# apache/incubator-predictionio

Measured on NVIDIA H100. Metric: ALS iterations/sec, higher is better.
Workload: dtype f32

## Files before the change

incubator-predictionio_b200/csrc/als_lockstep.cuh:

```cuda
#pragma once
#include <cuda_runtime.h>
#include <stdint.h>

namespace pio {

template <int N>
struct LsLayout {
  static constexpr int NBK = N / 16;
  static constexpr int NOFF = NBK * (NBK - 1) / 2;
  static constexpr int DIAG0 = NOFF * 256;
  static constexpr int SIZE = DIAG0 + NBK * 136;
  static constexpr int STRIDE = SIZE + ((SIZE % 32) == 16 ? 0 : (48 - SIZE % 32) % 32);
  __host__ __device__ static constexpr int swz(int rr) { return ((rr >> 1) & 1) * 2 + ((rr >> 2) & 1); }
  __host__ __device__ static constexpr int offd_base(int rb, int cb) { return (rb * (rb - 1) / 2 + cb) * 256; }
  __host__ __device__ static constexpr int offd(int rb, int cb, int rr, int cc) {
    return offd_base(rb, cb) + rr * 16 + 4 * ((cc >> 2) ^ swz(rr)) + (cc & 3);
  }
  __host__ __device__ static constexpr int diag(int rb, int rr, int cc) { return DIAG0 + rb * 136 + rr * (rr + 1) / 2 + cc; }
  __host__ __device__ static constexpr int at(int r, int c) {
    return (r >> 4) == (c >> 4) ? diag(r >> 4, r & 15, c & 15) : offd(r >> 4, c >> 4, r & 15, c & 15);
  }
};

__device__ __forceinline__ float ls_rsqrt(float x) {
  float r;
  asm("rsqrt.approx.ftz.f32 %0, %1;" : "=f"(r) : "f"(x));
  return r;
}

template <int N>
__device__ __forceinline__ void ls_add_yty(float* __restrict__ slot, const float* __restrict__ yty) {
  using LL = LsLayout<N>;
  const int lane = threadIdx.x & 31;
  for (int o = lane; o < LL::NOFF * 64; o += 32) {
    const int b = o >> 6, rr = (o >> 2) & 15, cg = o & 3;
    int rb = 1;
    while (rb * (rb + 1) / 2 <= b) ++rb;
    const int cb = b - rb * (rb - 1) / 2;
    float4* d = reinterpret_cast<float4*>(slot + LL::offd_base(rb, cb) + rr * 16 + 4 * (cg ^ LL::swz(rr)));
    const float4 y = __ldg(reinterpret_cast<const float4*>(yty + (size_t)(16 * rb + rr) * N + 16 * cb + 4 * cg));
    float4 v = *d;
    v.x += y.x; v.y += y.y; v.z += y.z; v.w += y.w;
    *d = v;
  }
  for (int o = lane; o < LL::NBK * 256; o += 32) {
    const int rb = o >> 8, rr = (o >> 4) & 15, cc = o & 15;
    if (cc <= rr) slot[LL::diag(rb, rr, cc)] += __ldg(yty + (size_t)(16 * rb + rr) * N + 16 * rb + cc);
  }
}

template <int N>
__device__ __forceinline__ void chol_lockstep(float* __restrict__ slot, const float* __restrict__ bvec, float ridge, int k,
                                              float* __restrict__ colbuf, float* __restrict__ dst_row, bool valid,
                                              int* __restrict__ fail) {
  using LL = LsLayout<N>;
  constexpr int LANES = N / 4;
  constexpr int Q = LANES / 16;
  constexpr int NBK = N / 16;
  static_assert(N == 64 || N == 128, "lockstep solver: N = 64 (two matrices per warp) or 128 (one)");
  const int lane = threadIdx.x & 31;
  const int l = lane % LANES, lq = l >> 4, lr = l & 15;
  const int sw = LL::swz(lr);
  float bb[4], yv[4], dv[4];
#pragma unroll
  for (int i = 0; i < 4; ++i) {
    bb[i] = bvec[i * LANES + l];
    yv[i] = 0.f;
    dv[i] = 0.f;
  }
  bool bad = false;
  __syncwarp();

#pragma unroll
  for (int p = 0; p < NBK; ++p) {
    constexpr int dummy = 0;
    (void)dummy;
    const int sp = p / Q;
    const bool isdiag = (Q == 1) || (lq == (p % Q));
    float a[4][16];
#pragma unroll
    for (int i = 0; i < 4; ++i) {
      if (i < sp) continue;
      const int bi = i * Q + lq;
      const int r = i * LANES + l;
      if (i == sp) {
#pragma unroll
        for (int c = 0; c < 16; ++c) {
          float v = 0.f;
          if (bi == p) {
            if (c <= lr) v = slot[LL::diag(p, lr, c)];
          } else if (bi > p) {
            v = slot[LL::offd(bi, p, lr, c)];
          }
          a[i][c] = v;
        }
      } else {
        const float* rowp = slot + LL::offd_base(bi, p) + lr * 16;
#pragma unroll
        for (int cg = 0; cg < 4; ++cg) {
          const float4 v = *reinterpret_cast<const float4*>(rowp + 4 * (cg ^ sw));
          a[i][4 * cg + 0] = v.x; a[i][4 * cg + 1] = v.y; a[i][4 * cg + 2] = v.z; a[i][4 * cg + 3] = v.w;
        }
      }
      if (i == sp) {
#pragma unroll
        for (int c = 0; c < 16; ++c)
          if (bi == p && c == lr) a[i][c] += ridge + (r >= k ? 1.f : 0.f);
      }
    }
    if (p > 0) {
#pragma unroll 1
      for (int q = 0; q < p; ++q) {
        const float* dblk = slot + LL::offd_base(p, q);
        const float* own[4];
#pragma unroll
        for (int i = 0; i < 4; ++i) {
          int bi = i * Q + lq;
          if (bi < p) bi = p;
          own[i] = slot + LL::offd_base(bi, q) + lr * 16;
        }
#pragma unroll 1
        for (int tg = 0; tg < 4; ++tg) {
          float4 o[4];
#pragma unroll
          for (int i = 0; i < 4; ++i)
            if (i >= sp) o[i] = *reinterpret_cast<const float4*>(own[i] + 4 * (tg ^ sw));
#pragma unroll
          for (int c = 0; c < 16; ++c) {
            const float4 d = *reinterpret_cast<const float4*>(dblk + c * 16 + 4 * (tg ^ LL::swz(c)));
#pragma unroll
            for (int i = 0; i < 4; ++i) {
              if (i < sp) continue;
              float v = a[i][c];
              v = fmaf(-o[i].x, d.x, v);
              v = fmaf(-o[i].y, d.y, v);
              v = fmaf(-o[i].z, d.z, v);
              v = fmaf(-o[i].w, d.w, v);
              a[i][c] = v;
            }
          }
        }
      }
    }
#pragma unroll
    for (int j = 0; j < 16; ++j) {
      float* cb = colbuf + (j & 1) * 32;
      if (isdiag) {
        cb[lr] = a[sp][j];
        cb[16 + lr] = bb[sp];
      }
      __syncwarp();
      float col[16];
#pragma unroll
      for (int cg = j / 4; cg < 4; ++cg) {
        const float4 v = *reinterpret_cast<const float4*>(cb + 4 * cg);
        col[4 * cg + 0] = v.x; col[4 * cg + 1] = v.y; col[4 * cg + 2] = v.z; col[4 * cg + 3] = v.w;
      }
      const float bg = cb[16 + j];
      float d = col[j];
      if (!(d > 0.f)) { bad = true; d = 1.f; }
      float inv = ls_rsqrt(d);
      inv = inv * (1.5f - 0.5f * d * inv * inv);
      const float inv2 = inv * inv;
      const float z = inv2 * bg;
      if (isdiag && lr == j) {
        yv[sp] = bg * inv;
        dv[sp] = inv;
      }
#pragma unroll
      for (int i = 0; i < 4; ++i) {
        if (i < sp) continue;
        const float aj = a[i][j];
        const float w = aj * inv2;
        if (i == sp) {
          const int bi = i * Q + lq;
          if (bi > p || (bi == p && lr > j)) bb[i] = fmaf(-aj, z, bb[i]);
        } else {
          bb[i] = fmaf(-aj, z, bb[i]);
        }
        a[i][j] = aj * inv;
#pragma unroll
        for (int c = j + 1; c < 16; ++c) a[i][c] = fmaf(-w, col[c], a[i][c]);
      }
    }
#pragma unroll
    for (int i = 0; i < 4; ++i) {
      if (i < sp) continue;
      const int bi = i * Q + lq;
      if (i == sp) {
#pragma unroll
        for (int c = 0; c < 16; ++c) {
          if (bi == p) {
            if (c <= lr) slot[LL::diag(p, lr, c)] = a[i][c];
          } else if (bi > p) {
            slot[LL::offd(bi, p, lr, c)] = a[i][c];
          }
        }
      } else {
        float* rowp = slot + LL::offd_base(bi, p) + lr * 16;
#pragma unroll
        for (int cg = 0; cg < 4; ++cg)
          *reinterpret_cast<float4*>(rowp + 4 * (cg ^ sw)) =
              make_float4(a[i][4 * cg + 0], a[i][4 * cg + 1], a[i][4 * cg + 2], a[i][4 * cg + 3]);
      }
    }
    __syncwarp();
  }

  float xs[4] = {0.f, 0.f, 0.f, 0.f};
#pragma unroll
  for (int g = N - 1; g >= 0; --g) {
    const int sg = g / LANES, lg = g % LANES, gb = g >> 4, gr = g & 15;
    const float t = yv[sg] * dv[sg];
    const float xg = __shfl_sync(0xffffffffu, t, lg, LANES);
    if (l == lg) xs[sg] = xg;
#pragma unroll
    for (int i = 0; i < 4; ++i) {
      if (i * Q > gb) continue;
      const int bi = i * Q + lq;
      if (bi < gb) yv[i] = fmaf(-slot[LL::offd(gb, bi, gr, lr)], xg, yv[i]);
      else if (bi == gb && lr < gr) yv[i] = fmaf(-slot[LL::diag(gb, gr, lr)], xg, yv[i]);
    }
  }
  if (valid) {
#pragma unroll
    for (int i = 0; i < 4; ++i) dst_row[i * LANES + l] = xs[i];
    if (bad && l == 0) atomicAdd(fail, 1);
  }
}

}
```

Before: 36.37.

## Software-pipeline Cholesky column updates and block the back-substitution per 16-row tile

The panel factorization now writes the next column into the shared column buffer immediately after updating only that column. The rest of the previous column's rank-1 update is deferred until after the next sync, shortening the serial warp-sync critical path per column. The back substitution replaces the per-element shuffle loop (N shuffles) with a per-16-block scheme: each block's diagonal triangle is solved redundantly by every lane from the buffer, and off-diagonal updates follow. This adds register pressure (pcol, x, y arrays) and redundant triangular work per lane, and output is written with float4 stores from lane 0.

```diff
diff --git a/incubator-predictionio_b200/csrc/als_lockstep.cuh b/incubator-predictionio_b200/csrc/als_lockstep.cuh
--- a/incubator-predictionio_b200/csrc/als_lockstep.cuh
+++ b/incubator-predictionio_b200/csrc/als_lockstep.cuh
@@ -142,13 +142,32 @@
         }
       }
     }
+    if (isdiag) {
+      colbuf[lr] = a[sp][0];
+      colbuf[16 + lr] = bb[sp];
+    }
+    float pcol[16], pinv = 0.f, pinv2 = 0.f, pz = 0.f, pw = 0.f;
+    auto rest = [&](int jj) {
+#pragma unroll
+      for (int i = 0; i < 4; ++i) {
+        if (i < sp) continue;
+        if (i == sp) {
+          a[i][jj] *= pinv;
+#pragma unroll
+          for (int c = jj + 2; c < 16; ++c) a[i][c] = fmaf(-pw, pcol[c], a[i][c]);
+        } else {
+          const float aj = a[i][jj];
+          const float w = aj * pinv2;
+          bb[i] = fmaf(-aj, pz, bb[i]);
+          a[i][jj] = aj * pinv;
+#pragma unroll
+          for (int c = jj + 1; c < 16; ++c) a[i][c] = fmaf(-w, pcol[c], a[i][c]);
+        }
+      }
+    };
 #pragma unroll
     for (int j = 0; j < 16; ++j) {
-      float* cb = colbuf + (j & 1) * 32;
-      if (isdiag) {
-        cb[lr] = a[sp][j];
-        cb[16 + lr] = bb[sp];
-      }
+      const float* cb = colbuf + (j & 1) * 32;
       __syncwarp();
       float col[16];
 #pragma unroll
@@ -157,6 +176,7 @@
         col[4 * cg + 0] = v.x; col[4 * cg + 1] = v.y; col[4 * cg + 2] = v.z; col[4 * cg + 3] = v.w;
       }
       const float bg = cb[16 + j];
+      if (j > 0) rest(j - 1);
       float d = col[j];
       if (!(d > 0.f)) { bad = true; d = 1.f; }
       float inv = ls_rsqrt(d);
@@ -167,22 +187,28 @@
         yv[sp] = bg * inv;
         dv[sp] = inv;
       }
-#pragma unroll
-      for (int i = 0; i < 4; ++i) {
-        if (i < sp) continue;
-        const float aj = a[i][j];
+      {
+        const int bi = sp * Q + lq;
+        const float aj = a[sp][j];
         const float w = aj * inv2;
-        if (i == sp) {
-          const int bi = i * Q + lq;
-          if (bi > p || (bi == p && lr > j)) bb[i] = fmaf(-aj, z, bb[i]);
-        } else {
-          bb[i] = fmaf(-aj, z, bb[i]);
-        }
-        a[i][j] = aj * inv;
-#pragma unroll
-        for (int c = j + 1; c < 16; ++c) a[i][c] = fmaf(-w, col[c], a[i][c]);
-      }
-    }
+        if (bi > p || (bi == p && lr > j)) bb[sp] = fmaf(-aj, z, bb[sp]);
+        if (j < 15) {
+          a[sp][j + 1] = fmaf(-w, col[j + 1], a[sp][j + 1]);
+          if (isdiag) {
+            float* nb = colbuf + ((j + 1) & 1) * 32;
+            nb[lr] = a[sp][j + 1];
+            nb[16 + lr] = bb[sp];
+          }
+        }
+        pw = w;
+      }
+#pragma unroll
+      for (int c = j; c < 16; ++c) pcol[c] = col[c];
+      pinv = inv;
+      pinv2 = inv2;
+      pz = z;
+    }
+    rest(15);
 #pragma unroll
     for (int i = 0; i < 4; ++i) {
       if (i < sp) continue;
@@ -207,26 +233,49 @@
     __syncwarp();
   }
 
-  float xs[4] = {0.f, 0.f, 0.f, 0.f};
-#pragma unroll
-  for (int g = N - 1; g >= 0; --g) {
-    const int sg = g / LANES, lg = g % LANES, gb = g >> 4, gr = g & 15;
-    const float t = yv[sg] * dv[sg];
-    const float xg = __shfl_sync(0xffffffffu, t, lg, LANES);
-    if (l == lg) xs[sg] = xg;
+#pragma unroll
+  for (int gb = NBK - 1; gb >= 0; --gb) {
+    const int sg = gb / Q;
+    float* line = colbuf + (gb & 1) * 32;
+    if ((Q == 1) || (lq == gb % Q)) {
+      line[lr] = yv[sg];
+      line[16 + lr] = dv[sg];
+    }
+    __syncwarp();
+    float y[16], dg[16], x[16];
+#pragma unroll
+    for (int cg = 0; cg < 4; ++cg) {
+      const float4 v = *reinterpret_cast<const float4*>(line + 4 * cg);
+      const float4 u = *reinterpret_cast<const float4*>(line + 16 + 4 * cg);
+      y[4 * cg + 0] = v.x; y[4 * cg + 1] = v.y; y[4 * cg + 2] = v.z; y[4 * cg + 3] = v.w;
+      dg[4 * cg + 0] = u.x; dg[4 * cg + 1] = u.y; dg[4 * cg + 2] = u.z; dg[4 * cg + 3] = u.w;
+    }
+    const float4* tri = reinterpret_cast<const float4*>(slot + LL::diag(gb, 0, 0));
+#pragma unroll
+    for (int r = 15; r >= 0; --r) {
+      x[r] = y[r] * dg[r];
+#pragma unroll
+      for (int c = 0; c < r; ++c) {
+        const int e = r * (r + 1) / 2 + c;
+        const float4 v = tri[e >> 2];
+        const float lv = (e & 3) == 0 ? v.x : (e & 3) == 1 ? v.y : (e & 3) == 2 ? v.z : v.w;
+        y[c] = fmaf(-lv, x[r], y[c]);
+      }
+    }
 #pragma unroll
     for (int i = 0; i < 4; ++i) {
-      if (i * Q > gb) continue;
       const int bi = i * Q + lq;
-      if (bi < gb) yv[i] = fmaf(-slot[LL::offd(gb, bi, gr, lr)], xg, yv[i]);
-      else if (bi == gb && lr < gr) yv[i] = fmaf(-slot[LL::diag(gb, gr, lr)], xg, yv[i]);
-    }
-  }
-  if (valid) {
-#pragma unroll
-    for (int i = 0; i < 4; ++i) dst_row[i * LANES + l] = xs[i];
-    if (bad && l == 0) atomicAdd(fail, 1);
-  }
-}
-
-}
+      if (i * Q > gb || bi >= gb) continue;
+#pragma unroll
+      for (int gr = 15; gr >= 0; --gr) yv[i] = fmaf(-slot[LL::offd(gb, bi, gr, lr)], x[gr], yv[i]);
+    }
+    if (valid && l == 0) {
+      float4* out = reinterpret_cast<float4*>(dst_row + 16 * gb);
+#pragma unroll
+      for (int cg = 0; cg < 4; ++cg) out[cg] = make_float4(x[4 * cg + 0], x[4 * cg + 1], x[4 * cg + 2], x[4 * cg + 3]);
+    }
+  }
+  if (valid && bad && l == 0) atomicAdd(fail, 1);
+}
+
+}
```

Result: no change. 36.45, median of 6 (+0.2%).
